# DeJhon-Huang/TrueTrace-Unity-Pathtracer

Hardware: AMD Instinct MI355X
Metric: Mrays/sec (primary+1-bounce) on Sponza CWBVH at 1080p; % HBM roofline (higher is better)
Workload: dtype f32

## Files before the change

truetrace-unity-pathtracer_amd/csrc/tt_trace.hip:

```cpp
#include "tt_launch.h"
#include "tt_wide.h"

#ifndef TT_LEAF_REFILL_MIN
#define TT_LEAF_REFILL_MIN (TT_LEAF_POOL ? 16 : TT_REFILL_MIN)
#endif

namespace {
template <int INFO, int LEAF = 0>
__device__ __forceinline__ bool write_record(const TraceArgs& A, uint32_t ray_index, uint32_t pix, float col_w,
                                             const Best& best, const LaneRay& wr, int32_t inst_mesh = 0,
                                             int32_t inst_tri_offset = 0) {
    tt_ray_data* R = A.rays + ray_index;
    const int32_t best_mesh = LEAF ? (best.tri_id != -1 ? inst_mesh : 0) : best.mesh_id;
    auto tri_offset_of_best = [&]() -> int32_t {
        if (LEAF) return best.tri_id != -1 ? inst_tri_offset : A.mesh[0].TriOffset;
        return A.mesh[best.mesh_id].TriOffset;
    };
    if (INFO != 0) {
        if (pix < A.n_pixels) {
            uint4 o;
            bool write = false;
            if (INFO == 1) {
                const int32_t to = tri_offset_of_best();
                o = make_uint4((uint32_t)best_mesh, (uint32_t)(best.tri_id - to),
                               __float_as_uint(best.u), __float_as_uint(best.v));
                write = true;
            } else {
                const float w = col_w;
                if (w == -1.0f || (float)A.bounce == w) {
                    write = true;
                    const bool miss = best.t == A.far_plane;
                    if ((A.flags & TT_TRACE_USE_RESTIRGI) && !miss) {
                        const int32_t to = tri_offset_of_best();
                        o.x = (uint32_t)best_mesh;
                        o.y = (uint32_t)(best.tri_id - to);
                        o.z = (uint32_t)(best.u * 65535.0f) | ((uint32_t)(best.v * 65535.0f) << 16);
                    } else {
                        LaneRay w = wr;
                        if (LEAF == 1) {
                            const uint4* rp = reinterpret_cast<const uint4*>(R);
                            const uint4 r0 = rp[0], r1 = rp[1];
                            w.ox = __uint_as_float(r0.x);
                            w.oy = __uint_as_float(r0.y);
                            w.oz = __uint_as_float(r0.z);
                            w.dx = __uint_as_float(r1.x);
                            w.dy = __uint_as_float(r1.y);
                            w.dz = __uint_as_float(r1.z);
                        }
                        if ((A.flags & TT_TRACE_USE_ASVGF) || !miss) {
                            o.x = __float_as_uint(w.dx);
                            o.y = __float_as_uint(w.dy);
                            o.z = __float_as_uint(w.dz);
                        } else {
                            o.x = __float_as_uint(w.dx * best.t + w.ox);
                            o.y = __float_as_uint(w.dy * best.t + w.oy);
                            o.z = __float_as_uint(w.dz * best.t + w.oz);
                        }
                    }
                    o.w = miss ? 1u : 0u;
                }
            }
            if (write) reinterpret_cast<uint4*>(A.info)[pix] = o;
        }
    }
    const uint32_t uv = (uint32_t)(best.u * 65535.0f) | ((uint32_t)(best.v * 65535.0f) << 16);
    const uint4 hit = make_uint4((uint32_t)best_mesh, (uint32_t)best.tri_id, __float_as_uint(best.t), uv);
    reinterpret_cast<uint4*>(R)[2] = hit;
    if (A.hits_out) {
        const u32x4 v = {hit.x, hit.y, hit.z, hit.w};
        __builtin_amdgcn_raw_buffer_store_b128(v, buffer_rsrc(A.hits_out, 0x7fffffff), (ray_index - A.ray_offset) << 4,
                                               0, 0);
    }
    return best.t != A.far_plane;
}

__device__ __forceinline__ void keep_record(const TraceArgs& A, uint32_t ray_index) {
    if (A.hits_out) {
        const uint4 h = reinterpret_cast<const uint4*>(A.rays + ray_index)[2];
        const u32x4 v = {h.x, h.y, h.z, h.w};
        __builtin_amdgcn_raw_buffer_store_b128(v, buffer_rsrc(A.hits_out, 0x7fffffff), (ray_index - A.ray_offset) << 4,
                                               0, 0);
    }
}

static_assert(TT_CHUNK_BIG == 64, "the adaptive order maps one dequeue (TT_CHUNK_BIG rays) to one 64-ray chunk");
#ifndef TT_ORDER_MIN_REPS
#define TT_ORDER_MIN_REPS 32
#endif
__device__ __forceinline__ void record_chunk_cost(const TraceArgs& A, bool swizzle, uint32_t ray_index, int32_t reps) {
    if (reps < TT_ORDER_MIN_REPS) return;
    const uint32_t local = ray_index - A.ray_offset;
    uint32_t c = local >> 6;
    if (swizzle) {
        const uint32_t py = fastdiv(local, A.div_width), px = local - py * A.width;
        c = (py >> 3) * (A.width >> 3) + (px >> 3);
    }
    atomicMax(A.chunk_cost + c, (uint32_t)reps);
}
}


namespace {
__device__ __forceinline__ bool root_leaf_hit(const RootLeaf& R, const LaneRay& r, float max_distance) {
    const float adjx = __uint_as_float(rl_byte(R.e, 0) << 23) * r.ix;
    const float adjy = __uint_as_float(rl_byte(R.e, 1) << 23) * r.iy;
    const float adjz = __uint_as_float(rl_byte(R.e, 2) << 23) * r.iz;
    const float orgx = r.ix * (R.px - r.ox);
    const float orgy = r.iy * (R.py - r.oy);
    const float orgz = r.iz * (R.pz - r.oz);
    const bool nx = r.dx < 0.0f, ny = r.dy < 0.0f, nz = r.dz < 0.0f;
    const uint32_t x_min = rl_byte(nx ? R.qhi : R.qlo, 0), x_max = rl_byte(nx ? R.qlo : R.qhi, 0);
    const uint32_t y_min = rl_byte(ny ? R.qhi : R.qlo, 1), y_max = rl_byte(ny ? R.qlo : R.qhi, 1);
    const uint32_t z_min = rl_byte(nz ? R.qhi : R.qlo, 2), z_max = rl_byte(nz ? R.qlo : R.qhi, 2);
    const float tminx = fma_((float)x_min, adjx, orgx);
    const float tminy = fma_((float)y_min, adjy, orgy);
    const float tminz = fma_((float)z_min, adjz, orgz);
    const float tmaxx = fma_((float)x_max, adjx, orgx);
    const float tmaxy = fma_((float)y_max, adjy, orgy);
    const float tmaxz = fma_((float)z_max, adjz, orgz);
    const float tmin = fmaxf(fmaxf(tminx, tminy), fmaxf(tminz, 1e-8f));
    float tmaxz_c;
    asm("v_min_f32 %0, %1, %2" : "=v"(tmaxz_c) : "v"(tmaxz), "v"(max_distance));
    const float tmax = fminf(fminf(tmaxx, tmaxy), tmaxz_c);
    return tmin < tmax;
}
}


template <bool STATS, bool MATCHECK, int INFO, bool IND, bool ORD, int LEAF = 0>
__device__ __forceinline__ void trace_body(const TraceArgs& A) {
    static_assert(!LEAF || (!STATS && !MATCHECK && !ORD), "the leaf-TLAS form has no stats / material / order variants");
    constexpr bool POOL = LEAF != 0 && TT_LEAF_POOL != 0;
    constexpr bool ROOTSTEP = POOL && TT_LEAF_ROOT_STEP != 0;
    constexpr int tt_lds_depth = lds_depth_of<LEAF>();
    static_assert(!POOL || TT_CHUNK_BIG == TT_WAVE, "the prepared-ray pool holds one chunk, one slot per lane");
    __shared__ uint2 s_stack[tt_lds_depth][TT_BLOCK];
    __shared__ uint4 s_pool[POOL ? 3 : 1][TT_BLOCK];
    (void)s_pool;
    LeafEntry L{};
    if (LEAF) L = load_leaf_mesh<true>(A.leaf, A.root.base_tri + firstbithigh(A.root.bits));
    uint32_t root_cg_x = 0, root_tg_x = 0, root_imask = 0;
    if (ROOTSTEP) {
        const NodeWords n = load_node_uniform(A.nodes, A.n_nodes, (uint32_t)L.off.w);
        root_cg_x = n.n1.x + (uint32_t)L.off.y;
        root_tg_x = n.n1.y + (uint32_t)L.off.x;
        root_imask = n.n0.w >> 24;
    }
    const uint32_t tid = threadIdx.x;
    zero_next_control(A.ctl_next, tid);
    const uint32_t gtid = blockIdx.x * TT_BLOCK + tid;
    const uint32_t spill_stride = gridDim.x * TT_BLOCK;
    uint2* __restrict__ spill = A.spill;
    (void)gtid;
    (void)spill_stride;
    (void)spill;
    const uint32_t lane = tid & (TT_WAVE - 1);
#ifdef TT_DIAG_BLOCKS
    if (tid < TT_DB_N) tt_db[tid] = 0ull;
    __syncthreads();
#endif

    uint32_t pool_next = 0, pool_end = 0, more = 1;
    const uint32_t wave_id = blockIdx.x * (TT_BLOCK / TT_WAVE) + (tid >> 6);
    SegState S{blockIdx.x % TT_SEGS, 0u, 0u};
    const uint32_t n_rays = IND ? launch_ray_count(A) : A.n_rays;
    const uint32_t n_tiles = (n_rays + 63u) >> 6;
    const bool swizzle = IND ? (A.tile_swizzle && n_rays == A.n_pixels) : (A.tile_swizzle != 0u);
    const __amdgpu_buffer_rsrc_t nodes = buffer_rsrc(A.nodes, A.n_nodes * (uint32_t)TT_NODE_STRIDE);
    const __amdgpu_buffer_rsrc_t tris = buffer_rsrc(A.tris, A.n_tris * (uint32_t)sizeof(TriPos));

    constexpr uint32_t TT_IDLE = 0x80000000u;
    uint32_t ray_index = 0;
    uint32_t pix = 0;
    float col_w = 0.0f;
    bool pending = false;
    LaneRay ray{}, wray{};
    Best best{};
    uint2 cg = make_uint2(0u, 0u), tg = make_uint2(0u, TT_IDLE);
    uint32_t oct = 0;
    int32_t stack_size = 0, tlas_ss = -1;
    int32_t NodeOffset = 0, TriOffset = 0, MatOffset = 0, mesh_id = -1, Reps = 0;
    if (LEAF) {
        NodeOffset = L.off.y;
        TriOffset = L.off.x;
        MatOffset = L.off.z;
        mesh_id = L.mesh_id;
    }
    uint32_t c_nodes = 0, c_tris = 0, c_blas = 0, c_acc = 0, c_rays = 0, c_hits = 0, c_reps = 0, c_ovf = 0;
    uint32_t d_iter = 0, d_node_lanes = 0, d_node_iters = 0, d_tri_lanes = 0, d_tri_iters = 0, d_active_lanes = 0;
    uint32_t d_lead_same = 0, d_uniform = 0;
    auto world_ray = [&]() -> LaneRay { return wray; };
    auto ray_of = [&](uint32_t widx) -> uint32_t {
        uint32_t local = widx;
        if (swizzle) {
            const uint32_t tw = A.width >> 3;
            const uint32_t t = widx >> 6, l = widx & 63u;
            const uint32_t ty = fastdiv(t, A.div_tiles), tx = t - ty * tw;
            local = (ty * 8u + (l >> 3)) * A.width + tx * 8u + (l & 7u);
        }
        return A.ray_offset + local;
    };
    (void)ray_of;

#if TT_ROOT_LEAF
    const bool rl_ok = A.root.ok != 0u;
#endif
    auto enter_blas = [&]() {
            TT_DB(8);
            const uint32_t mo = firstbithigh(tg.y);
            tg.y &= ~(1u << mo);
            const LeafEntry e = load_leaf_mesh<true>(A.leaf, tg.x + mo);
            mesh_id = e.mesh_id;
            NodeOffset = e.off.y;
            TriOffset = e.off.x;
            bool ok = true;
            if (tg.y != 0u) TT_PUSH(tg, ok);
            if (ok && (cg.y & 0xff000000u)) TT_PUSH(cg, ok);
            tg.y = 0u;
            if (ok) {
                tlas_ss = stack_size;
                MatOffset = e.off.z;
                enter_object_space(e, ray, oct, cg);
                if (STATS) c_blas++;
            } else {
                tg.y = TT_IDLE;
                if (STATS) c_ovf++;
                TT_REPORT_OVERFLOW(A);
                keep_record(A, ray_index);
            }
    };
    auto finish_ray = [&]() {
        const bool hit = write_record<INFO, LEAF>(A, ray_index, pix, col_w, best, world_ray(), mesh_id, TriOffset);
        if (STATS) c_hits += hit ? 1u : 0u;
        (void)hit;
        if (ORD) record_chunk_cost(A, swizzle, ray_index, Reps);
    };
    constexpr uint32_t REFILL_MIN = LEAF ? TT_LEAF_REFILL_MIN : TT_REFILL_MIN;
    while (true) {
        TT_DB(0);
        const uint64_t idle = __ballot((int32_t)tg.y < 0);
        const uint32_t n_idle = (uint32_t)__builtin_popcount((uint32_t)idle) + (uint32_t)__builtin_popcount((uint32_t)(idle >> 32));
        const bool pool_dry = !more && pool_next >= pool_end;
#if TT_DRAIN_PRIO
        if (pool_dry) __builtin_amdgcn_s_setprio(TT_DRAIN_PRIO);
#endif
        const bool to_wide = TT_WIDE && pool_dry && n_idle < TT_WAVE && TT_WAVE - n_idle <= TT_WIDE_ENTER;
        if ((n_idle == TT_WAVE && pool_dry) || (n_idle >= REFILL_MIN && !pool_dry) || to_wide) {
            if (pending) {
                TT_DB(1);
                finish_ray();
                pending = false;
            }
        }
        if (n_idle == TT_WAVE && pool_dry) break;
#if TT_WIDE
        if (to_wide) {
            TT_DB(13);
            WideState st{{ray, world_ray(), cg, tg, oct, stack_size, tlas_ss, NodeOffset, TriOffset, MatOffset, Reps,
                          ray_index, tid, gtid, (int32_t)tg.y >= 0},
                         best, mesh_id, pix, col_w};
            regroup<2, LEAF>(st, __ballot((int32_t)tg.y >= 0), lane);
            auto finish_wide = [&](const WideState& w) {
                const bool hit = write_record<INFO, LEAF>(A, w.ray_index, w.pix, w.col_w, w.best, w.wray, mesh_id, TriOffset);
                if (STATS) c_hits += hit ? 1u : 0u;
                if (ORD) record_chunk_cost(A, swizzle, w.ray_index, w.Reps);
            };
            auto exhaust_wide = [&](const WideState& w) {
                keep_record(A, w.ray_index);
                if (ORD) record_chunk_cost(A, swizzle, w.ray_index, w.Reps);
            };
            wide_phase<STATS, MATCHECK, 2, LEAF>(A, st, s_stack, spill, spill_stride, nodes, tris, lane,
                                           Counters{c_nodes, c_tris, c_blas, c_acc, c_hits, c_reps, c_ovf},
                                           finish_wide, exhaust_wide);
            break;
        }
#endif
        if (n_idle >= REFILL_MIN && !pool_dry) {
            TT_DB(2);
#if TT_LONG_PRIO
            if (__ballot((int32_t)tg.y >= 0 && Reps >= TT_LONG_PRIO) != 0ull) __builtin_amdgcn_s_setprio(TT_LONG_PRIO_LEVEL);
            else __builtin_amdgcn_s_setprio(0);
#endif
            const uint32_t avail = pool_end - pool_next;
            uint32_t new_base = 0, new_count = 0;
            if (avail < n_idle && more) {
                new_count = sched_reserve(A.ctl, n_rays, n_tiles, lane, n_idle - avail, wave_id, S, new_base);
                more = new_count > 0 ? 1u : 0u;
                if (ORD && A.order && new_count > 0)
                    new_base = (__builtin_amdgcn_readfirstlane(A.order[new_base >> 6]) << 6) | (new_base & 63u);
            }
            const PoolTake pt = pool_take<TT_UNIFORM_POOL != 0>(idle, n_idle, new_base, new_count, pool_next, pool_end, more);
            const uint32_t widx = pt.widx;
            pool_next = pt.pool_next;
            pool_end = pt.pool_end;
            more = pt.more;
            if constexpr (POOL) {
                const uint32_t pcol = tid - lane;
                const bool take = (int32_t)tg.y < 0 && widx != 0xffffffffu;
                const bool take_left = take && lane_prefix(idle) < min(avail, n_idle);
                auto start_ray = [&](const uint4 p0, const uint4 p1, const uint4 p2) {
                    TT_DL(19, true);
                    ray_index = ray_of(widx);
                    ray.ox = __uint_as_float(p0.x);
                    ray.oy = __uint_as_float(p0.y);
                    ray.oz = __uint_as_float(p0.z);
                    ray.dx = __uint_as_float(p0.w);
                    ray.dy = __uint_as_float(p1.x);
                    ray.dz = __uint_as_float(p1.y);
                    ray.ix = __uint_as_float(p1.z);
                    ray.iy = __uint_as_float(p1.w);
                    ray.iz = __uint_as_float(p2.x);
                    pix = p2.y;
                    if (ROOTSTEP) {
                        col_w = -1.0f;
                        oct = p2.z & 0x7fffffffu;
                        const uint32_t inner = p2.w & 0xff000000u;
                        cg = make_uint2(root_cg_x, inner ? (inner | root_imask) : 0u);
                        tg = make_uint2(root_tg_x, p2.w & 0x00ffffffu);
                        Reps = (p2.z & 0x80000000u) ? 2 : 1;
                    } else {
                        col_w = __uint_as_float(p2.z);
                        oct = p2.w & 0x7fffffffu;
                        cg = make_uint2((p2.w & 0x80000000u) ? (uint32_t)L.off.w : 0u, p2.w & 0x80000000u);
                    }
                    if (LEAF == 2) {
                        const uint4* rp = reinterpret_cast<const uint4*>(A.rays + ray_index);
                        const uint4 r0 = rp[0], r1 = rp[1];
                        wray.ox = __uint_as_float(r0.x);
                        wray.oy = __uint_as_float(r0.y);
                        wray.oz = __uint_as_float(r0.z);
                        wray.dx = __uint_as_float(r1.x);
                        wray.dy = __uint_as_float(r1.y);
                        wray.dz = __uint_as_float(r1.z);
                    }
                    best.t = A.far_plane;
                    best.u = 0.0f;
                    best.v = 0.0f;
                    best.mesh_id = 0;
                    best.tri_id = -1;
                    if (!ROOTSTEP) tg = make_uint2(0u, 0u);
                    stack_size = 0;
                    if (!ROOTSTEP) Reps = 1;
                };
                uint4 p0 = make_uint4(0u, 0u, 0u, 0u), p1 = p0, p2 = p0;
                if (take_left) {
                    const uint32_t slot = pcol + (widx & 63u);
                    p0 = s_pool[0][slot];
                    p1 = s_pool[1][slot];
                    p2 = s_pool[2][slot];
                    if (ROOTSTEP) start_ray(p0, p1, p2);
                }
                __builtin_amdgcn_fence(__ATOMIC_ACQ_REL, "wavefront");
                __builtin_amdgcn_wave_barrier();
                if (new_count > 0) {
                    TT_DB(4);
                    uint4 q0 = make_uint4(0u, 0u, 0u, 0u), q1 = q0, q2 = q0;
                    NodeWords rn{};
                    if (ROOTSTEP) rn = load_node_uniform(A.nodes, A.n_nodes, (uint32_t)L.off.w);
                    if (lane < new_count) {
                        const uint4* rp = reinterpret_cast<const uint4*>(A.rays + ray_of(new_base + lane));
                        const uint4 r0 = rp[0], r1 = rp[1];
                        float cw = 0.0f;
                        if (INFO == 2) cw = (r0.w < A.n_pixels) ? A.colors[r0.w].Data[3] : 0.0f;
                        LaneRay r;
                        r.ox = __uint_as_float(r0.x);
                        r.oy = __uint_as_float(r0.y);
                        r.oz = __uint_as_float(r0.z);
                        r.dx = __uint_as_float(r1.x);
                        r.dy = __uint_as_float(r1.y);
                        r.dz = __uint_as_float(r1.z);
                        r.ix = rcp_rn(r.dx);
                        r.iy = rcp_rn(r.dy);
                        r.iz = rcp_rn(r.dz);
                        uint32_t o = 0u;
                        uint2 g = make_uint2(0u, 0u);
                        const bool root_hit = root_leaf_hit(A.root, r, A.far_plane);
                        TT_DL(29, root_hit);
                        if (root_hit) enter_object_space(L, r, o, g);
                        q0 = make_uint4(__float_as_uint(r.ox), __float_as_uint(r.oy), __float_as_uint(r.oz),
                                        __float_as_uint(r.dx));
                        q1 = make_uint4(__float_as_uint(r.dy), __float_as_uint(r.dz), __float_as_uint(r.ix),
                                        __float_as_uint(r.iy));
                        q2 = make_uint4(__float_as_uint(r.iz), r0.w, __float_as_uint(cw), o | g.y);
                        if (ROOTSTEP) {
                            if (INFO == 2 && !(cw == -1.0f || (float)A.bounce == cw)) q2.y = 0xffffffffu;
                            q2.z = o | g.y;
                            q2.w = 0u;
                            s_pool[0][tid] = q0;
                            s_pool[1][tid] = q1;
                            s_pool[2][tid] = q2;
                            if (root_hit) {
                                TT_DB(28);
                                s_pool[2][tid].w = node_intersect(rn.n0, rn.n1, rn.n2, rn.n3, rn.n4, r, o, A.far_plane);
                            }
                        }
                    }
                    if (!ROOTSTEP) {
                        s_pool[0][tid] = q0;
                        s_pool[1][tid] = q1;
                        s_pool[2][tid] = q2;
                    }
                }
                __builtin_amdgcn_fence(__ATOMIC_ACQ_REL, "wavefront");
                __builtin_amdgcn_wave_barrier();
                if (take && !take_left) {
                    const uint32_t slot = pcol + (widx & 63u);
                    p0 = s_pool[0][slot];
                    p1 = s_pool[1][slot];
                    p2 = s_pool[2][slot];
                    if (ROOTSTEP) start_ray(p0, p1, p2);
                }
                if (!ROOTSTEP && take) start_ray(p0, p1, p2);
            }
            if (!POOL && (int32_t)tg.y < 0 && widx != 0xffffffffu) {
                TT_DB(4);
                TT_DL(19, true);
                uint32_t local = widx;
                if (swizzle) {
                    const uint32_t tw = A.width >> 3;
                    const uint32_t t = widx >> 6, l = widx & 63u;
                    const uint32_t ty = fastdiv(t, A.div_tiles), tx = t - ty * tw;
                    local = (ty * 8u + (l >> 3)) * A.width + tx * 8u + (l & 7u);
                }
                ray_index = A.ray_offset + local;
                const uint4* rp = reinterpret_cast<const uint4*>(A.rays + ray_index);
                const uint4 r0 = rp[0], r1 = rp[1];
                pix = r0.w;
                if (INFO == 2) col_w = (pix < A.n_pixels) ? A.colors[pix].Data[3] : 0.0f;
                ray.ox = __uint_as_float(r0.x);
                ray.oy = __uint_as_float(r0.y);
                ray.oz = __uint_as_float(r0.z);
                ray.dx = __uint_as_float(r1.x);
                ray.dy = __uint_as_float(r1.y);
                ray.dz = __uint_as_float(r1.z);
                ray.ix = rcp_rn(ray.dx);
                ray.iy = rcp_rn(ray.dy);
                ray.iz = rcp_rn(ray.dz);
                best.t = A.far_plane;
                best.u = 0.0f;
                best.v = 0.0f;
                best.mesh_id = 0;
                best.tri_id = -1;
                tg = make_uint2(0u, 0u);
                stack_size = 0;
                if (LEAF) {
                    if (LEAF == 2) wray = ray;
                    cg = make_uint2(0u, 0u);
                    Reps = 1;
                    if (root_leaf_hit(A.root, ray, best.t)) enter_object_space(L, ray, oct, cg);
                }
                if (!LEAF) {
                    wray = ray;
                    oct = octant_inv4(ray);
                    cg = make_uint2(A.tlas_base, 0x80000000u);
                    tlas_ss = -1;
                    NodeOffset = (int32_t)A.tlas_base;
                    TriOffset = 0;
                    MatOffset = 0;
                    mesh_id = -1;
                    Reps = 0;
                }
                if (STATS) c_rays++;
#if TT_ROOT_LEAF
                if (!LEAF && rl_ok) {
                    const RootLeaf& RL = A.root;
                    const bool hit = root_leaf_hit(RL, ray, best.t);
                    cg = make_uint2(RL.base_child, 0u);
                    tg = make_uint2(RL.base_tri, hit ? RL.bits : 0u);
                    Reps = 1;
                    if (STATS) c_nodes++;
                    if (hit) enter_blas();
                }
#endif
            }
        }

        if (STATS) {
            const uint64_t nm = __ballot(tg.y == 0u && Reps < TT_MAX_REPS && (cg.y & 0xff000000u));
            const uint64_t am = __ballot((int32_t)tg.y >= 0);
            if (lane == 0) {
                d_iter++;
                d_node_lanes += (uint32_t)__popcll(nm);
                d_node_iters += nm ? 1u : 0u;
                d_active_lanes += (uint32_t)__popcll(am);
            }
        }
        if (tg.y == 0u) {
            TT_DB(5);
            if (Reps >= TT_MAX_REPS) {
                tg.y = TT_IDLE;
                if (STATS) c_reps++;
                keep_record(A, ray_index);
                if (ORD) record_chunk_cost(A, swizzle, ray_index, Reps);
            } else if (cg.y & 0xff000000u) {
                const uint32_t child = take_child(cg, oct);
                bool ok = true;
                if (cg.y & 0xff000000u) {
                    TT_DB(7);
                    TT_PUSH(cg, ok);
                }
                if (ok) {
                    TT_DB(6);
                    TT_DL(17, true);
                    if (STATS) {
                        const uint32_t lead = __builtin_amdgcn_readfirstlane(child);
                        const uint64_t same = __ballot(child == lead), all = __ballot(true);
                        d_lead_same += child == lead ? 1u : 0u;
                        d_uniform += (same == all && lane == (uint32_t)__builtin_ctzll(all)) ? 1u : 0u;
                    }
                    const NodeWords n = load_node<TT_NODE_CPOL>(nodes, child);
                    const uint32_t hitmask = node_intersect(n.n0, n.n1, n.n2, n.n3, n.n4, ray, oct, best.t);
                    cg = node_group(hitmask, n, NodeOffset);
                    tg = tri_group(hitmask, n, TriOffset);
                    Reps++;
                    if (STATS) c_nodes++;
                } else {
                    tg.y = TT_IDLE;
                    if (STATS) c_ovf++;
                    TT_REPORT_OVERFLOW(A);
                    keep_record(A, ray_index);
                }
            } else {
                tg = cg;
                cg = make_uint2(0u, 0u);
            }
            if (!LEAF && (int32_t)tg.y > 0 && tlas_ss == -1) enter_blas();
        }

        if (STATS) {
            const uint64_t tm = __ballot((int32_t)tg.y > 0);
            if (lane == 0) {
                d_tri_lanes += (uint32_t)__popcll(tm);
                d_tri_iters += tm ? 1u : 0u;
            }
        }
        if ((int32_t)tg.y > 0) {
            TT_DB(9);
            TT_DL(18, true);
            const uint32_t ti = firstbithigh(tg.y);
            tg.y &= ~(1u << ti);
            const bool acc = intersect_triangle<MATCHECK>(tris, A.mat, A.bounce == 0, A.flags, (int32_t)(tg.x + ti),
                                                          mesh_id, MatOffset, ray, best);
            if (STATS) {
                c_tris++;
                c_acc += acc ? 1u : 0u;
            }
        }

        if (tg.y == 0u && (cg.y & 0xff000000u) == 0u) {
            TT_DB(10);
            if (stack_size != 0) {
                TT_DB(11);
                if (!LEAF && stack_size == tlas_ss) {
                    TT_DB(12);
                    leave_blas(A.tlas_base, world_ray(), NodeOffset, TriOffset, tlas_ss, ray, oct);
                }
                TT_POP(cg);
            } else {
                pending = true;
                tg.y = TT_IDLE;
            }
        }
    }

#ifdef TT_DIAG_BLOCKS
    __syncthreads();
    if (tid < TT_DB_N && A.diag_times && tt_db[tid]) atomicAdd(A.diag_times + tid, tt_db[tid]);
#endif
    if (STATS) {
        const uint32_t v[8] = {wave_sum(c_rays), wave_sum(c_nodes), wave_sum(c_tris), wave_sum(c_blas),
                               wave_sum(c_hits), wave_sum(c_reps), wave_sum(c_ovf), wave_sum(c_acc)};
        if (lane == 0) {
#pragma unroll
            for (int k = 0; k < 8; k++)
                if (v[k]) atomicAdd(&A.ctl->stats[k], (unsigned long long)v[k]);
            const uint32_t d[6] = {d_iter, d_node_iters, d_node_lanes, d_tri_iters, d_tri_lanes, d_active_lanes};
#pragma unroll
            for (int k = 0; k < 6; k++) atomicAdd(&A.ctl->diag[k], (unsigned long long)d[k]);
        }
        const uint32_t ls = wave_sum(d_lead_same), un = wave_sum(d_uniform);
        if (lane == 0) {
            atomicAdd(&A.ctl->diag[6], (unsigned long long)ls);
            atomicAdd(&A.ctl->diag[7], (unsigned long long)un);
        }
    }
}

template <bool STATS, bool MATCHECK, int INFO>
__global__ TT_BOUNDS void tt_trace_kernel(TraceArgs A) {
    trace_body<STATS, MATCHECK, INFO, false, false>(A);
}
template <bool MATCHECK, int INFO>
__global__ TT_BOUNDS void tt_trace_kernel_indirect(TraceArgs A) {
    trace_body<false, MATCHECK, INFO, true, false>(A);
}
template <int INFO>
__global__ __launch_bounds__(TT_BLOCK) __attribute__((amdgpu_waves_per_eu(5))) void tt_trace_kernel_ord(TraceArgs A) {
    trace_body<false, false, INFO, false, true>(A);
}
template <int INFO>
__global__ TT_BOUNDS void tt_trace_kernel_ord_mat(TraceArgs A) {
    trace_body<false, true, INFO, false, true>(A);
}
#ifndef TT_LEAF_WAVES
#define TT_LEAF_WAVES(INFO) 6
#endif
#define TT_LEAF_BOUNDS __launch_bounds__(TT_BLOCK) __attribute__((amdgpu_waves_per_eu(TT_LEAF_WAVES(INFO))))
#ifndef TT_LEAF_WRAY_RESIDENT
#define TT_LEAF_WRAY_RESIDENT 1
#endif
#define TT_LEAF_FORM(INFO) ((INFO) == 2 && TT_LEAF_WRAY_RESIDENT ? 2 : 1)
template <bool IND, int INFO>
__global__ TT_LEAF_BOUNDS void tt_trace_leaf_kernel(TraceArgs A) {
    trace_body<false, false, INFO, IND, false, TT_LEAF_FORM(INFO)>(A);
}

template <bool S, bool M, int I>
static hipError_t launch_one(const TraceArgs& a, bool leaf, uint32_t grid, hipStream_t st) {
    if constexpr (!S && !M) {
        if (leaf) {
            if (a.n_rays_dev) hipLaunchKernelGGL((tt_trace_leaf_kernel<true, I>), dim3(grid), dim3(TT_BLOCK), 0, st, a);
            else hipLaunchKernelGGL((tt_trace_leaf_kernel<false, I>), dim3(grid), dim3(TT_BLOCK), 0, st, a);
            return hipGetLastError();
        }
    }
    if constexpr (!S) {
        if (a.n_rays_dev) {
            hipLaunchKernelGGL((tt_trace_kernel_indirect<M, I>), dim3(grid), dim3(TT_BLOCK), 0, st, a);
            return hipGetLastError();
        }
        if (a.chunk_cost) {
            if (M) hipLaunchKernelGGL((tt_trace_kernel_ord_mat<I>), dim3(grid), dim3(TT_BLOCK), 0, st, a);
            else hipLaunchKernelGGL((tt_trace_kernel_ord<I>), dim3(grid), dim3(TT_BLOCK), 0, st, a);
            return hipGetLastError();
        }
    }
    hipLaunchKernelGGL((tt_trace_kernel<S, M, I>), dim3(grid), dim3(TT_BLOCK), 0, st, a);
    return hipGetLastError();
}

template <bool S, bool M>
static hipError_t launch_info(const TraceArgs& a, int info, bool leaf, uint32_t grid, hipStream_t st) {
    if (info == 0) return launch_one<S, M, 0>(a, leaf, grid, st);
    if (info == 1) return launch_one<S, M, 1>(a, leaf, grid, st);
    return launch_one<S, M, 2>(a, leaf, grid, st);
}

hipError_t tt_launch_trace(const TraceArgs& a, bool stats, bool matcheck, int info, bool leaf, uint32_t grid,
                           hipStream_t st) {
    if (leaf && (stats || matcheck || a.chunk_cost || !root_one_instance(a.root))) return hipErrorInvalidValue;
    if (stats)
        return matcheck ? launch_info<true, true>(a, info, false, grid, st) : launch_info<true, false>(a, info, false, grid, st);
    return matcheck ? launch_info<false, true>(a, info, false, grid, st) : launch_info<false, false>(a, info, leaf, grid, st);
}

hipError_t tt_trace_occupancy_table(int* out24) {
    out24[0] = occupancy_of(tt_trace_kernel<false, false, 0>);
    out24[1] = occupancy_of(tt_trace_kernel<false, false, 1>);
    out24[2] = occupancy_of(tt_trace_kernel<false, false, 2>);
    out24[3] = occupancy_of(tt_trace_kernel<false, true, 0>);
    out24[4] = occupancy_of(tt_trace_kernel<false, true, 1>);
    out24[5] = occupancy_of(tt_trace_kernel<false, true, 2>);
    out24[6] = occupancy_of(tt_trace_kernel<true, false, 0>);
    out24[7] = occupancy_of(tt_trace_kernel<true, false, 1>);
    out24[8] = occupancy_of(tt_trace_kernel<true, false, 2>);
    out24[9] = occupancy_of(tt_trace_kernel<true, true, 0>);
    out24[10] = occupancy_of(tt_trace_kernel<true, true, 1>);
    out24[11] = occupancy_of(tt_trace_kernel<true, true, 2>);
    out24[12] = occupancy_of(tt_trace_kernel_ord<0>);
    out24[13] = occupancy_of(tt_trace_kernel_ord<1>);
    out24[14] = occupancy_of(tt_trace_kernel_ord<2>);
    out24[15] = occupancy_of(tt_trace_kernel_ord_mat<0>);
    out24[16] = occupancy_of(tt_trace_kernel_ord_mat<1>);
    out24[17] = occupancy_of(tt_trace_kernel_ord_mat<2>);
    out24[18] = occupancy_of(tt_trace_leaf_kernel<false, 0>);
    out24[19] = occupancy_of(tt_trace_leaf_kernel<false, 1>);
    out24[20] = occupancy_of(tt_trace_leaf_kernel<false, 2>);
    out24[21] = occupancy_of(tt_trace_leaf_kernel<true, 0>);
    out24[22] = occupancy_of(tt_trace_leaf_kernel<true, 1>);
    out24[23] = occupancy_of(tt_trace_leaf_kernel<true, 2>);
    return hipGetLastError();
}

uint32_t tt_trace_block_size() { return TT_BLOCK; }
uint32_t tt_trace_chunk_rays() { return TT_CHUNK_BIG; }
uint32_t tt_trace_lds_bytes(bool leaf) {
    const uint32_t stack = (uint32_t)((leaf ? lds_depth_of<1>() : lds_depth_of<0>()) * TT_BLOCK * sizeof(uint2));
    return stack + (leaf && TT_LEAF_POOL ? (uint32_t)(3 * TT_BLOCK * sizeof(uint4)) : 0u);
}
uint32_t tt_trace_spill_entries() {
    constexpr int depth = lds_depth_of<1>() < lds_depth_of<0>() ? lds_depth_of<1>() : lds_depth_of<0>();
    return depth >= TT_STACK_SIZE ? 0u : (uint32_t)(TT_STACK_SIZE - depth);
}
```

truetrace-unity-pathtracer_amd/csrc/tt_traverse.h:

```cpp
#ifndef TT_TRAVERSE_H
#define TT_TRAVERSE_H
#include "tt_device.h"

#define TT_WAVE 64
#ifndef TT_BLOCK
#define TT_BLOCK 64
#endif
#ifndef TT_SEGS
#define TT_SEGS 8
#endif
#ifndef TT_CHUNK_BIG
#define TT_CHUNK_BIG 64
#endif
#ifndef TT_REFILL_MIN
#define TT_REFILL_MIN 20
#endif
#ifndef TT_PUSH_FAST
#define TT_PUSH_FAST 1
#endif
#ifndef TT_DRAIN_PRIO
#define TT_DRAIN_PRIO 2
#endif
#ifndef TT_LONG_PRIO
#define TT_LONG_PRIO 64
#endif
#ifndef TT_LONG_PRIO_LEVEL
#define TT_LONG_PRIO_LEVEL 2
#endif
#ifndef TT_UNIFORM_POOL
#define TT_UNIFORM_POOL 1
#endif
#ifndef TT_LDS_STACK
#define TT_LDS_STACK 12
#endif
#ifndef TT_LEAF_POOL
#define TT_LEAF_POOL 1
#endif
#ifndef TT_LEAF_LDS_STACK
#define TT_LEAF_LDS_STACK 6
#endif
#ifndef TT_LEAF_ROOT_STEP
#define TT_LEAF_ROOT_STEP 1
#endif
#ifndef TT_WAVES_PER_EU
#define TT_WAVES_PER_EU 0
#endif
#if TT_WAVES_PER_EU > 0
#define TT_BOUNDS __launch_bounds__(TT_BLOCK, TT_WAVES_PER_EU)
#else
#define TT_BOUNDS __launch_bounds__(TT_BLOCK)
#endif

#ifdef TT_DIAG_BLOCKS
#define TT_DB_N 32
__shared__ unsigned long long tt_db[TT_DB_N];
#define TT_DB(k)                                                                               \
    do {                                                                                       \
        const uint64_t m_ = __ballot(1);                                                       \
        if ((threadIdx.x & 63u) == (uint32_t)__builtin_ctzll(m_)) atomicAdd(&tt_db[k], 1ull); \
    } while (0)
#define TT_DL(k, pred)                                                                         \
    do {                                                                                       \
        const uint64_t p_ = __ballot(pred), m_ = __ballot(1);                                  \
        if ((threadIdx.x & 63u) == (uint32_t)__builtin_ctzll(m_))                              \
            atomicAdd(&tt_db[k], (unsigned long long)__popcll(p_));                            \
    } while (0)
#else
#define TT_DB(k) \
    do {         \
    } while (0)
#define TT_DL(k, pred) \
    do {               \
    } while (0)
#endif

namespace {

struct LaneRay {
    float ox, oy, oz, dx, dy, dz, ix, iy, iz;
};

__device__ __forceinline__ float fma_(float a, float b, float c) { return __builtin_fmaf(a, b, c); }
__device__ __forceinline__ uint32_t firstbithigh(uint32_t x) { return 31u - (uint32_t)__builtin_clz(x); }

__device__ __forceinline__ uint32_t octant_inv4(const LaneRay& r) {
    return (r.dx < 0.0f ? 0u : 0x04040404u) | (r.dy < 0.0f ? 0u : 0x02020202u) |
           (r.dz < 0.0f ? 0u : 0x01010101u);
}


typedef uint32_t u32x4 __attribute__((ext_vector_type(4)));
__device__ __forceinline__ __amdgpu_buffer_rsrc_t buffer_rsrc(const void* base, uint32_t bytes) {
    return __builtin_amdgcn_make_buffer_rsrc(const_cast<void*>(base), 0, (int)bytes, 0x00020000);
}
#ifndef TT_TRI_CPOL
#define TT_TRI_CPOL 0
#endif
#ifndef TT_NODE_CPOL
#define TT_NODE_CPOL 0
#endif
template <int CPOL = 0>
__device__ __forceinline__ uint4 buffer_load16(__amdgpu_buffer_rsrc_t r, uint32_t off) {
    const u32x4 v = __builtin_amdgcn_raw_buffer_load_b128(r, off, 0, CPOL);
    return make_uint4(v.x, v.y, v.z, v.w);
}
typedef uint32_t u32x2 __attribute__((ext_vector_type(2)));
template <int CPOL = 0>
__device__ __forceinline__ uint2 buffer_load8(__amdgpu_buffer_rsrc_t r, uint32_t off) {
    const u32x2 v = __builtin_amdgcn_raw_buffer_load_b64(r, off, 0, CPOL);
    return make_uint2(v.x, v.y);
}
template <int CPOL = 0>
__device__ __forceinline__ uint32_t buffer_load4(__amdgpu_buffer_rsrc_t r, uint32_t off) {
    return __builtin_amdgcn_raw_buffer_load_b32(r, off, 0, CPOL);
}
static_assert(TT_NODE_STRIDE == 80 || TT_NODE_STRIDE == 128, "node stride: 80 (the reference array) or 128");
__device__ __forceinline__ uint32_t node_offset(uint32_t i) {
    if (TT_NODE_STRIDE == 128) return i << 7;
    uint32_t r;
    asm("v_lshl_add_u32 %0, %1, 2, %1\n\tv_lshlrev_b32 %0, 4, %0" : "=&v"(r) : "v"(i));
    return r;
}
__device__ __forceinline__ uint32_t tri_offset(uint32_t i) {
    uint32_t r;
    asm("v_lshl_add_u32 %0, %1, 1, %1\n\tv_lshlrev_b32 %0, 4, %0" : "=&v"(r) : "v"(i));
    return r;
}

__device__ __forceinline__ uint32_t node_intersect(const uint4 n0, const uint4 n1, const uint4 n2,
                                                   const uint4 n3, const uint4 n4, const LaneRay& r,
                                                   uint32_t oct_inv4, float max_distance) {
    const uint32_t w = n0.w;
    uint32_t ex, ey, ez;
    asm("v_lshlrev_b32_sdwa %0, %1, %2 dst_sel:DWORD dst_unused:UNUSED_PAD src0_sel:DWORD src1_sel:BYTE_0"
        : "=v"(ex) : "s"(23u), "v"(w));
    asm("v_lshlrev_b32_sdwa %0, %1, %2 dst_sel:DWORD dst_unused:UNUSED_PAD src0_sel:DWORD src1_sel:BYTE_1"
        : "=v"(ey) : "s"(23u), "v"(w));
    asm("v_lshlrev_b32_sdwa %0, %1, %2 dst_sel:DWORD dst_unused:UNUSED_PAD src0_sel:DWORD src1_sel:BYTE_2"
        : "=v"(ez) : "s"(23u), "v"(w));
    const float adjx = __uint_as_float(ex) * r.ix;
    const float adjy = __uint_as_float(ey) * r.iy;
    const float adjz = __uint_as_float(ez) * r.iz;
    const float orgx = r.ix * (__uint_as_float(n0.x) - r.ox);
    const float orgy = r.iy * (__uint_as_float(n0.y) - r.oy);
    const float orgz = r.iz * (__uint_as_float(n0.z) - r.oz);
    const bool nx = r.dx < 0.0f, ny = r.dy < 0.0f, nz = r.dz < 0.0f;
    uint32_t hit_mask = 0;
#pragma unroll
    for (int i = 0; i < 2; i++) {
        const uint32_t meta4 = i == 0 ? n1.z : n1.w;
        const uint32_t is_inner4 = (meta4 & (meta4 << 1)) & 0x10101010u;
        const uint32_t inner_mask4 = (is_inner4 >> 1) - (is_inner4 >> 4);
        const uint32_t bit_index4 = (meta4 ^ (oct_inv4 & inner_mask4)) & 0x1f1f1f1fu;
        const uint32_t child_bits4 = (meta4 >> 5) & 0x07070707u;
        const uint32_t qlx = i == 0 ? n2.x : n2.y, qhx = i == 0 ? n2.z : n2.w;
        const uint32_t qly = i == 0 ? n3.x : n3.y, qhy = i == 0 ? n3.z : n3.w;
        const uint32_t qlz = i == 0 ? n4.x : n4.y, qhz = i == 0 ? n4.z : n4.w;
        const uint32_t x_min = nx ? qhx : qlx, x_max = nx ? qlx : qhx;
        const uint32_t y_min = ny ? qhy : qly, y_max = ny ? qly : qhy;
        const uint32_t z_min = nz ? qhz : qlz, z_max = nz ? qlz : qhz;
#pragma unroll
        for (int j = 0; j < 4; j++) {
            const float tminx = fma_((float)((x_min >> (j * 8)) & 0xffu), adjx, orgx);
            const float tminy = fma_((float)((y_min >> (j * 8)) & 0xffu), adjy, orgy);
            const float tminz = fma_((float)((z_min >> (j * 8)) & 0xffu), adjz, orgz);
            const float tmaxx = fma_((float)((x_max >> (j * 8)) & 0xffu), adjx, orgx);
            const float tmaxy = fma_((float)((y_max >> (j * 8)) & 0xffu), adjy, orgy);
            const float tmaxz = fma_((float)((z_max >> (j * 8)) & 0xffu), adjz, orgz);
            const float tmin = fmaxf(fmaxf(tminx, tminy), fmaxf(tminz, 1e-8f));
            float tmaxz_c;
            asm("v_min_f32 %0, %1, %2" : "=v"(tmaxz_c) : "v"(tmaxz), "v"(max_distance));
            const float tmax = fminf(fminf(tmaxx, tmaxy), tmaxz_c);
            uint32_t bits;
            if (j == 0)
                asm("v_lshlrev_b32_sdwa %0, %1, %2 dst_sel:DWORD dst_unused:UNUSED_PAD src0_sel:BYTE_0 src1_sel:BYTE_0"
                    : "=v"(bits) : "v"(bit_index4), "v"(child_bits4));
            else if (j == 1)
                asm("v_lshlrev_b32_sdwa %0, %1, %2 dst_sel:DWORD dst_unused:UNUSED_PAD src0_sel:BYTE_1 src1_sel:BYTE_1"
                    : "=v"(bits) : "v"(bit_index4), "v"(child_bits4));
            else if (j == 2)
                asm("v_lshlrev_b32_sdwa %0, %1, %2 dst_sel:DWORD dst_unused:UNUSED_PAD src0_sel:BYTE_2 src1_sel:BYTE_2"
                    : "=v"(bits) : "v"(bit_index4), "v"(child_bits4));
            else
                asm("v_lshlrev_b32_sdwa %0, %1, %2 dst_sel:DWORD dst_unused:UNUSED_PAD src0_sel:BYTE_3 src1_sel:BYTE_3"
                    : "=v"(bits) : "v"(bit_index4), "v"(child_bits4));
            hit_mask |= (tmin < tmax) ? bits : 0u;
        }
    }
    return hit_mask;
}


__device__ __forceinline__ uint32_t take_child(uint2& cg, uint32_t oct) {
    const uint32_t cio = firstbithigh(cg.y);
    const uint32_t slot = (cio - 24u) ^ (oct & 0xffu);
    const uint32_t rel = __builtin_popcount(cg.y & ~(0xffffffffu << slot));
    const uint32_t child = cg.x + rel;
    cg.y &= ~(1u << cio);
    return child;
}
struct NodeWords {
    uint4 n0, n1, n2, n3, n4;
};
template <int CPOL>
__device__ __forceinline__ NodeWords load_node(__amdgpu_buffer_rsrc_t nodes, uint32_t child) {
    const uint32_t no = node_offset(child);
    return NodeWords{buffer_load16<CPOL>(nodes, no), buffer_load16<CPOL>(nodes, no + 16u),
                     buffer_load16<CPOL>(nodes, no + 32u), buffer_load16<CPOL>(nodes, no + 48u),
                     buffer_load16<CPOL>(nodes, no + 64u)};
}
__device__ __forceinline__ NodeWords load_node_uniform(const uint4* nodes, uint32_t n_nodes, uint32_t node) {
    u32x4 a = {0u, 0u, 0u, 0u}, b = a, c = a, d = a, e = a;
    if (node < n_nodes) {
        const char* p = reinterpret_cast<const char*>(nodes) + (size_t)node * TT_NODE_STRIDE;
        asm volatile("s_nop 4\n\t"
                     "s_load_dwordx4 %0, %5, 0x0\n\t"
                     "s_load_dwordx4 %1, %5, 0x10\n\t"
                     "s_load_dwordx4 %2, %5, 0x20\n\t"
                     "s_load_dwordx4 %3, %5, 0x30\n\t"
                     "s_load_dwordx4 %4, %5, 0x40\n\t"
                     "s_waitcnt lgkmcnt(0)"
                     : "=&s"(a), "=&s"(b), "=&s"(c), "=&s"(d), "=&s"(e)
                     : "s"(p));
    }
    return NodeWords{make_uint4(a.x, a.y, a.z, a.w), make_uint4(b.x, b.y, b.z, b.w), make_uint4(c.x, c.y, c.z, c.w),
                     make_uint4(d.x, d.y, d.z, d.w), make_uint4(e.x, e.y, e.z, e.w)};
}
__device__ __forceinline__ uint2 node_group(uint32_t hitmask, const NodeWords& n, int32_t NodeOffset) {
    return make_uint2(n.n1.x + (uint32_t)NodeOffset, (hitmask & 0xff000000u) | (n.n0.w >> 24));
}
__device__ __forceinline__ uint2 tri_group(uint32_t hitmask, const NodeWords& n, int32_t TriOffset) {
    return make_uint2(n.n1.y + (uint32_t)TriOffset, hitmask & 0x00ffffffu);
}

struct LeafEntry {
    float4 m0, m1, m2;
    int4 off;
    int32_t mesh_id;
};
template <bool MESH_ID>
__device__ __forceinline__ LeafEntry load_leaf_mesh(const LeafMesh* leaf, uint32_t i) {
    const float4* mp = reinterpret_cast<const float4*>(leaf + i);
    LeafEntry e;
    e.m0 = mp[0];
    e.m1 = mp[1];
    e.m2 = mp[2];
    e.off = reinterpret_cast<const int4*>(mp)[3];
    e.mesh_id = MESH_ID ? reinterpret_cast<const int4*>(mp)[4].x : 0;
    return e;
}
__device__ __forceinline__ LaneRay to_object_space(const float4 m0, const float4 m1, const float4 m2, const LaneRay& ray) {
    LaneRay nr;
    nr.dx = fma_(m0.z, ray.dz, fma_(m0.y, ray.dy, m0.x * ray.dx));
    nr.dy = fma_(m1.z, ray.dz, fma_(m1.y, ray.dy, m1.x * ray.dx));
    nr.dz = fma_(m2.z, ray.dz, fma_(m2.y, ray.dy, m2.x * ray.dx));
    nr.ox = fma_(m0.z, ray.oz, fma_(m0.y, ray.oy, m0.x * ray.ox)) + m0.w;
    nr.oy = fma_(m1.z, ray.oz, fma_(m1.y, ray.oy, m1.x * ray.ox)) + m1.w;
    nr.oz = fma_(m2.z, ray.oz, fma_(m2.y, ray.oy, m2.x * ray.ox)) + m2.w;
    nr.ix = rcp_rn(nr.dx);
    nr.iy = rcp_rn(nr.dy);
    nr.iz = rcp_rn(nr.dz);
    return nr;
}
__device__ __forceinline__ void enter_object_space(const LeafEntry& e, LaneRay& ray, uint32_t& oct, uint2& cg) {
    ray = to_object_space(e.m0, e.m1, e.m2, ray);
    oct = octant_inv4(ray);
    cg = make_uint2((uint32_t)e.off.w, 0x80000000u);
}
__device__ __forceinline__ void leave_blas(uint32_t tlas_base, const LaneRay& wray, int32_t& NodeOffset,
                                           int32_t& TriOffset, int32_t& tlas_ss, LaneRay& ray, uint32_t& oct) {
    NodeOffset = (int32_t)tlas_base;
    TriOffset = 0;
    tlas_ss = -1;
    ray = wray;
    oct = octant_inv4(ray);
}

struct Best {
    float t, u, v;
    int32_t mesh_id, tri_id;
};

__device__ __forceinline__ float2 align_uv(float bu, float bv, const int32_t* tex, const float* scale) {
    if (tex[0] <= 0) return make_float2(-1.0f, -1.0f);
    const float dx = (float)(((uint32_t)tex[0]) & 0x7FFFu) / 16384.0f;
    const float dy = (float)(((uint32_t)tex[0]) >> 15) / 16384.0f;
    const float dz = (float)(((uint32_t)tex[1]) & 0x7FFFu) / 16384.0f;
    const float dw = (float)(((uint32_t)tex[1]) >> 15) / 16384.0f;
    float x = bu * scale[0] + scale[2];
    float y = bv * scale[1] + scale[3];
    x = x < 0.0f ? 1.0f - fmodf(fabsf(x), 1.0f) : fmodf(fabsf(x), 1.0f);
    y = y < 0.0f ? 1.0f - fmodf(fabsf(y), 1.0f) : fmodf(fabsf(y), 1.0f);
    return make_float2(x * (dx - dz) + dz, y * (dy - dw) + dw);
}
__device__ __forceinline__ float2 align_uv(float2 b, const CutoutMat& m) { return align_uv(b.x, b.y, m.alpha_tex, m.scale); }
__device__ __forceinline__ int atlas_clamp(float c, uint32_t n) { return (int)fminf(fmaxf(c, 0.0f), (float)(n - 1u)); }
__device__ __forceinline__ float atlas_texel(const MatView& M, int x, int y) {
    return (float)M.atlas[(size_t)y * M.atlas_w + (size_t)x] / 255.0f;
}
__device__ __forceinline__ float sample_point(const MatView& M, float2 uv) {
    return atlas_texel(M, atlas_clamp(floorf(uv.x * (float)M.atlas_w), M.atlas_w),
                       atlas_clamp(floorf(uv.y * (float)M.atlas_h), M.atlas_h));
}
__device__ __forceinline__ float sample_linear(const MatView& M, float2 uv) {
    const float x = uv.x * (float)M.atlas_w - 0.5f, y = uv.y * (float)M.atlas_h - 0.5f;
    const float x0 = floorf(x), y0 = floorf(y);
    const float fx = x - x0, fy = y - y0;
    const int ix0 = atlas_clamp(x0, M.atlas_w), ix1 = atlas_clamp(x0 + 1.0f, M.atlas_w);
    const int iy0 = atlas_clamp(y0, M.atlas_h), iy1 = atlas_clamp(y0 + 1.0f, M.atlas_h);
    const float a = atlas_texel(M, ix0, iy0) * (1.0f - fx) + atlas_texel(M, ix1, iy0) * fx;
    const float b = atlas_texel(M, ix0, iy1) * (1.0f - fx) + atlas_texel(M, ix1, iy1) * fx;
    return a * (1.0f - fy) + b * fy;
}
__device__ __forceinline__ float half_bits_to_float(uint32_t h) {
    return (float)__builtin_bit_cast(_Float16, (uint16_t)h);
}
__device__ __forceinline__ float3 sample_tex_point(const MatView& M, float2 uv) {
    const int x = atlas_clamp(floorf(uv.x * (float)M.tex_w), M.tex_w);
    const int y = atlas_clamp(floorf(uv.y * (float)M.tex_h), M.tex_h);
    const uint2 t = M.tex[(size_t)y * M.tex_w + (size_t)x];
    return make_float3(half_bits_to_float(t.x & 0xffffu), half_bits_to_float(t.x >> 16),
                       half_bits_to_float(t.y & 0xffffu));
}
__device__ __forceinline__ float3 glass_tint(const MatView& M, const GlassMat& g, float2 buv) {
    const float3 x = sample_tex_point(M, align_uv(buv.x, buv.y, g.albedo_tex, g.scale));
    return make_float3((g.color[0] * (x.x + 2.0f)) / 3.0f, (g.color[1] * (x.y + 2.0f)) / 3.0f,
                       (g.color[2] * (x.z + 2.0f)) / 3.0f);
}

__device__ __forceinline__ float2 base_uv(const MatView& M, int32_t tri_id, float u, float v) {
    const float2* t = reinterpret_cast<const float2*>(reinterpret_cast<const char*>(M.raw + tri_id) + 60);
    const float2 t0 = t[0], t1 = t[1], t2 = t[2];
    const float w = 1.0f - u - v;
    return make_float2(t0.x * w + t1.x * u + t2.x * v, t0.y * w + t1.y * u + t2.y * v);
}

struct TriCand {
    float t, u, v;
    bool cand, accept;
};
struct TriData {
    uint4 a, b;
    uint2 c;
};
template <bool MATCHECK, int CPOL = TT_TRI_CPOL>
__device__ __forceinline__ TriData triangle_load(__amdgpu_buffer_rsrc_t tris, int32_t tri_id) {
    const uint32_t to = tri_offset((uint32_t)tri_id);
    TriData d;
    d.a = buffer_load16<CPOL>(tris, to);
    d.b = buffer_load16<CPOL>(tris, to + 16u);
    if (MATCHECK) {
        d.c = buffer_load8<CPOL>(tris, to + 32u);
    } else {
        d.c.x = buffer_load4<CPOL>(tris, to + 32u);
        d.c.y = 0u;
    }
    return d;
// ... 227 lines not shown
```

Before: 7514.

## Restart finished leaf-form lanes inline from the ray pool, parking their hits

In the leaf-TLAS pool path, lanes whose traversal finishes now immediately take the next prepared ray from the LDS pool inside the traversal loop. They stash their finished hit (tri, t, u, v, ray index, pixel) in the consumed pool slot and write it out at the next refill point. This aims to cut idle-lane time between refills and raise SIMD utilisation. In exchange it adds per-iteration ballots and LDS traffic, and it disables the resident world-ray form (LEAF=2) when restart is on.

New measurement: 7727, median of 6. 2.8% higher.

```diff
diff --git a/truetrace-unity-pathtracer_amd/csrc/tt_trace.hip b/truetrace-unity-pathtracer_amd/csrc/tt_trace.hip
--- a/truetrace-unity-pathtracer_amd/csrc/tt_trace.hip
+++ b/truetrace-unity-pathtracer_amd/csrc/tt_trace.hip
@@ -132,6 +132,8 @@
     static_assert(!LEAF || (!STATS && !MATCHECK && !ORD), "the leaf-TLAS form has no stats / material / order variants");
     constexpr bool POOL = LEAF != 0 && TT_LEAF_POOL != 0;
     constexpr bool ROOTSTEP = POOL && TT_LEAF_ROOT_STEP != 0;
+    constexpr bool RESTART = ROOTSTEP && TT_LEAF_RESTART != 0;
+    static_assert(!RESTART || LEAF == 1, "the restart parks no world ray: the record write reads it back");
     constexpr int tt_lds_depth = lds_depth_of<LEAF>();
     static_assert(!POOL || TT_CHUNK_BIG == TT_WAVE, "the prepared-ray pool holds one chunk, one slot per lane");
     __shared__ uint2 s_stack[tt_lds_depth][TT_BLOCK];
@@ -201,6 +203,12 @@
         return A.ray_offset + local;
     };
     (void)ray_of;
+    uint64_t parked = 0ull;
+    (void)parked;
+    auto ray_index_of = [&](uint32_t v) -> uint32_t {
+        if constexpr (RESTART) return ray_of(v);
+        return v;
+    };
 
 #if TT_ROOT_LEAF
     const bool rl_ok = A.root.ok != 0u;
@@ -230,11 +238,57 @@
             }
     };
     auto finish_ray = [&]() {
-        const bool hit = write_record<INFO, LEAF>(A, ray_index, pix, col_w, best, world_ray(), mesh_id, TriOffset);
+        const bool hit = write_record<INFO, LEAF>(A, ray_index_of(ray_index), pix, col_w, best, world_ray(), mesh_id,
+                                                  TriOffset);
         if (STATS) c_hits += hit ? 1u : 0u;
         (void)hit;
         if (ORD) record_chunk_cost(A, swizzle, ray_index, Reps);
     };
+    auto start_from = [&](const uint32_t widx, const uint4 p0, const uint4 p1, const uint4 p2) {
+        TT_DL(19, true);
+        ray_index = RESTART ? widx : ray_of(widx);
+        ray.ox = __uint_as_float(p0.x);
+        ray.oy = __uint_as_float(p0.y);
+        ray.oz = __uint_as_float(p0.z);
+        ray.dx = __uint_as_float(p0.w);
+        ray.dy = __uint_as_float(p1.x);
+        ray.dz = __uint_as_float(p1.y);
+        ray.ix = __uint_as_float(p1.z);
+        ray.iy = __uint_as_float(p1.w);
+        ray.iz = __uint_as_float(p2.x);
+        pix = p2.y;
+        if (ROOTSTEP) {
+            col_w = -1.0f;
+            oct = p2.z & 0x7fffffffu;
+            const uint32_t inner = p2.w & 0xff000000u;
+            cg = make_uint2(root_cg_x, inner ? (inner | root_imask) : 0u);
+            tg = make_uint2(root_tg_x, p2.w & 0x00ffffffu);
+            Reps = (p2.z & 0x80000000u) ? 2 : 1;
+        } else {
+            col_w = __uint_as_float(p2.z);
+            oct = p2.w & 0x7fffffffu;
+            cg = make_uint2((p2.w & 0x80000000u) ? (uint32_t)L.off.w : 0u, p2.w & 0x80000000u);
+        }
+        if (LEAF == 2) {
+            const uint4* rp = reinterpret_cast<const uint4*>(A.rays + ray_index);
+            const uint4 r0 = rp[0], r1 = rp[1];
+            wray.ox = __uint_as_float(r0.x);
+            wray.oy = __uint_as_float(r0.y);
+            wray.oz = __uint_as_float(r0.z);
+            wray.dx = __uint_as_float(r1.x);
+            wray.dy = __uint_as_float(r1.y);
+            wray.dz = __uint_as_float(r1.z);
+        }
+        best.t = A.far_plane;
+        best.u = 0.0f;
+        best.v = 0.0f;
+        best.mesh_id = 0;
+        best.tri_id = -1;
+        if (!ROOTSTEP) tg = make_uint2(0u, 0u);
+        stack_size = 0;
+        if (!ROOTSTEP) Reps = 1;
+    };
+    (void)start_from;
     constexpr uint32_t REFILL_MIN = LEAF ? TT_LEAF_REFILL_MIN : TT_REFILL_MIN;
     while (true) {
         TT_DB(0);
@@ -245,11 +299,32 @@
         if (pool_dry) __builtin_amdgcn_s_setprio(TT_DRAIN_PRIO);
 #endif
         const bool to_wide = TT_WIDE && pool_dry && n_idle < TT_WAVE && TT_WAVE - n_idle <= TT_WIDE_ENTER;
-        if ((n_idle == TT_WAVE && pool_dry) || (n_idle >= REFILL_MIN && !pool_dry) || to_wide) {
+        const uint32_t refill_min = RESTART && pool_next >= pool_end ? (uint32_t)TT_LEAF_RESTART_MIN : REFILL_MIN;
+        if ((n_idle == TT_WAVE && pool_dry) || (n_idle >= refill_min && !pool_dry) || to_wide) {
             if (pending) {
                 TT_DB(1);
                 finish_ray();
                 pending = false;
+            }
+            if constexpr (RESTART) {
+                if (parked != 0ull) {
+                    TT_DB(34);
+                    if ((parked >> lane) & 1ull) {
+                        TT_DL(35, true);
+                        const uint4 k0 = s_pool[0][tid];
+                        const uint2 k1 = reinterpret_cast<const uint2*>(&s_pool[1][tid])[0];
+                        Best kb;
+                        kb.tri_id = (int32_t)k0.x;
+                        kb.t = __uint_as_float(k0.y);
+                        kb.u = __uint_as_float(k0.z);
+                        kb.v = __uint_as_float(k0.w);
+                        kb.mesh_id = 0;
+                        write_record<INFO, LEAF>(A, ray_of(k1.x), k1.y, -1.0f, kb, LaneRay{}, mesh_id, TriOffset);
+                    }
+                    parked = 0ull;
+                    __builtin_amdgcn_fence(__ATOMIC_ACQ_REL, "wavefront");
+                    __builtin_amdgcn_wave_barrier();
+                }
             }
         }
         if (n_idle == TT_WAVE && pool_dry) break;
@@ -257,7 +332,7 @@
         if (to_wide) {
             TT_DB(13);
             WideState st{{ray, world_ray(), cg, tg, oct, stack_size, tlas_ss, NodeOffset, TriOffset, MatOffset, Reps,
-                          ray_index, tid, gtid, (int32_t)tg.y >= 0},
+                          ray_index_of(ray_index), tid, gtid, (int32_t)tg.y >= 0},
                          best, mesh_id, pix, col_w};
             regroup<2, LEAF>(st, __ballot((int32_t)tg.y >= 0), lane);
             auto finish_wide = [&](const WideState& w) {
@@ -275,7 +350,7 @@
             break;
         }
 #endif
-        if (n_idle >= REFILL_MIN && !pool_dry) {
+        if (n_idle >= refill_min && !pool_dry) {
             TT_DB(2);
 #if TT_LONG_PRIO
             if (__ballot((int32_t)tg.y >= 0 && Reps >= TT_LONG_PRIO) != 0ull) __builtin_amdgcn_s_setprio(TT_LONG_PRIO_LEVEL);
@@ -298,50 +373,7 @@
                 const uint32_t pcol = tid - lane;
                 const bool take = (int32_t)tg.y < 0 && widx != 0xffffffffu;
                 const bool take_left = take && lane_prefix(idle) < min(avail, n_idle);
-                auto start_ray = [&](const uint4 p0, const uint4 p1, const uint4 p2) {
-                    TT_DL(19, true);
-                    ray_index = ray_of(widx);
-                    ray.ox = __uint_as_float(p0.x);
-                    ray.oy = __uint_as_float(p0.y);
-                    ray.oz = __uint_as_float(p0.z);
-                    ray.dx = __uint_as_float(p0.w);
-                    ray.dy = __uint_as_float(p1.x);
-                    ray.dz = __uint_as_float(p1.y);
-                    ray.ix = __uint_as_float(p1.z);
-                    ray.iy = __uint_as_float(p1.w);
-                    ray.iz = __uint_as_float(p2.x);
-                    pix = p2.y;
-                    if (ROOTSTEP) {
-                        col_w = -1.0f;
-                        oct = p2.z & 0x7fffffffu;
-                        const uint32_t inner = p2.w & 0xff000000u;
-                        cg = make_uint2(root_cg_x, inner ? (inner | root_imask) : 0u);
-                        tg = make_uint2(root_tg_x, p2.w & 0x00ffffffu);
-                        Reps = (p2.z & 0x80000000u) ? 2 : 1;
-                    } else {
-                        col_w = __uint_as_float(p2.z);
-                        oct = p2.w & 0x7fffffffu;
-                        cg = make_uint2((p2.w & 0x80000000u) ? (uint32_t)L.off.w : 0u, p2.w & 0x80000000u);
-                    }
-                    if (LEAF == 2) {
-                        const uint4* rp = reinterpret_cast<const uint4*>(A.rays + ray_index);
-                        const uint4 r0 = rp[0], r1 = rp[1];
-                        wray.ox = __uint_as_float(r0.x);
-                        wray.oy = __uint_as_float(r0.y);
-                        wray.oz = __uint_as_float(r0.z);
-                        wray.dx = __uint_as_float(r1.x);
-                        wray.dy = __uint_as_float(r1.y);
-                        wray.dz = __uint_as_float(r1.z);
-                    }
-                    best.t = A.far_plane;
-                    best.u = 0.0f;
-                    best.v = 0.0f;
-                    best.mesh_id = 0;
-                    best.tri_id = -1;
-                    if (!ROOTSTEP) tg = make_uint2(0u, 0u);
-                    stack_size = 0;
-                    if (!ROOTSTEP) Reps = 1;
-                };
+                auto start_ray = [&](const uint4 p0, const uint4 p1, const uint4 p2) { start_from(widx, p0, p1, p2); };
                 uint4 p0 = make_uint4(0u, 0u, 0u, 0u), p1 = p0, p2 = p0;
                 if (take_left) {
                     const uint32_t slot = pcol + (widx & 63u);
@@ -475,6 +507,7 @@
             }
         }
 
+        TT_DL(30, (int32_t)tg.y < 0);
         if (STATS) {
             const uint64_t nm = __ballot(tg.y == 0u && Reps < TT_MAX_REPS && (cg.y & 0xff000000u));
             const uint64_t am = __ballot((int32_t)tg.y >= 0);
@@ -490,7 +523,7 @@
             if (Reps >= TT_MAX_REPS) {
                 tg.y = TT_IDLE;
                 if (STATS) c_reps++;
-                keep_record(A, ray_index);
+                keep_record(A, ray_index_of(ray_index));
                 if (ORD) record_chunk_cost(A, swizzle, ray_index, Reps);
             } else if (cg.y & 0xff000000u) {
                 const uint32_t child = take_child(cg, oct);
@@ -518,7 +551,7 @@
                     tg.y = TT_IDLE;
                     if (STATS) c_ovf++;
                     TT_REPORT_OVERFLOW(A);
-                    keep_record(A, ray_index);
+                    keep_record(A, ray_index_of(ray_index));
                 }
             } else {
                 tg = cg;
@@ -547,8 +580,53 @@
             }
         }
 
-        if (tg.y == 0u && (cg.y & 0xff000000u) == 0u) {
+        if constexpr (RESTART) {
+            const bool used_up = tg.y == 0u && (cg.y & 0xff000000u) == 0u;
+            const bool finishing = used_up && stack_size == 0;
+            if (used_up) {
+                TT_DB(10);
+                TT_DL(31, finishing);
+                if (stack_size != 0) {
+                    TT_DB(11);
+                    TT_POP(cg);
+                }
+            }
+            const uint64_t fin = __ballot(finishing);
+            if (fin != 0ull) {
+                TT_DB(32);
+                const uint32_t n_fin = (uint32_t)__builtin_popcount((uint32_t)fin) + (uint32_t)__builtin_popcount((uint32_t)(fin >> 32));
+                const uint32_t n_take = min(n_fin, pool_end - pool_next);
+                if (finishing) {
+                    const uint32_t rank = lane_prefix(fin);
+                    if (rank < n_take) {
+                        TT_DL(33, true);
+                        const uint32_t widx = pool_next + rank;
+                        const uint32_t slot = (tid - lane) + (widx & 63u);
+                        const uint4 p0 = s_pool[0][slot], p1 = s_pool[1][slot], p2 = s_pool[2][slot];
+#ifdef TT_TEST_PARK_SWAP
+                        s_pool[0][slot] = make_uint4((uint32_t)best.tri_id, __float_as_uint(best.t), __float_as_uint(best.v),
+                                                     __float_as_uint(best.u));
+#else
+                        s_pool[0][slot] = make_uint4((uint32_t)best.tri_id, __float_as_uint(best.t), __float_as_uint(best.u),
+                                                     __float_as_uint(best.v));
+#endif
+                        reinterpret_cast<uint2*>(&s_pool[1][slot])[0] = make_uint2(ray_index, pix);
+                        start_from(widx, p0, p1, p2);
+                    } else {
+                        pending = true;
+                        tg.y = TT_IDLE;
+                    }
+                }
+                if (n_take != 0u) {
+                    const uint64_t m = n_take >= 64u ? ~0ull : ((1ull << n_take) - 1ull);
+                    parked |= m << (pool_next & 63u);
+                    pool_next += n_take;
+                }
+            }
+        } else if (tg.y == 0u && (cg.y & 0xff000000u) == 0u) {
             TT_DB(10);
+            TT_DL(31, stack_size == 0);
+            if (stack_size == 0) TT_DB(32);
             if (stack_size != 0) {
                 TT_DB(11);
                 if (!LEAF && stack_size == tlas_ss) {
@@ -609,7 +687,8 @@
 #ifndef TT_LEAF_WRAY_RESIDENT
 #define TT_LEAF_WRAY_RESIDENT 1
 #endif
-#define TT_LEAF_FORM(INFO) ((INFO) == 2 && TT_LEAF_WRAY_RESIDENT ? 2 : 1)
+#define TT_LEAF_FORM(INFO) \
+    ((INFO) == 2 && TT_LEAF_WRAY_RESIDENT && !(TT_LEAF_POOL && TT_LEAF_ROOT_STEP && TT_LEAF_RESTART) ? 2 : 1)
 template <bool IND, int INFO>
 __global__ TT_LEAF_BOUNDS void tt_trace_leaf_kernel(TraceArgs A) {
     trace_body<false, false, INFO, IND, false, TT_LEAF_FORM(INFO)>(A);
diff --git a/truetrace-unity-pathtracer_amd/csrc/tt_traverse.h b/truetrace-unity-pathtracer_amd/csrc/tt_traverse.h
--- a/truetrace-unity-pathtracer_amd/csrc/tt_traverse.h
+++ b/truetrace-unity-pathtracer_amd/csrc/tt_traverse.h
@@ -41,6 +41,12 @@
 #endif
 #ifndef TT_LEAF_ROOT_STEP
 #define TT_LEAF_ROOT_STEP 1
+#endif
+#ifndef TT_LEAF_RESTART
+#define TT_LEAF_RESTART 1
+#endif
+#ifndef TT_LEAF_RESTART_MIN
+#define TT_LEAF_RESTART_MIN 16
 #endif
 #ifndef TT_WAVES_PER_EU
 #define TT_WAVES_PER_EU 0
@@ -52,7 +58,7 @@
 #endif
 
 #ifdef TT_DIAG_BLOCKS
-#define TT_DB_N 32
+#define TT_DB_N 40
 __shared__ unsigned long long tt_db[TT_DB_N];
 #define TT_DB(k)                                                                               \
     do {                                                                                       \
```
